# facebookresearch/flashy

Measured on AMD Instinct MI355X. Metric: img/sec, higher is better.
Workload: dtype bf16; 1 GPU; model=resnet18, dataset=cifar10-shaped, global_batch=64, img_size=32, num_classes=10, parallelism=dp1, mode=native-kernels, graph=True, channels_last=False

## Files before the change

flashy_amd/models/resnet_native.py:

```python
from __future__ import annotations

import typing as tp

import torch
from torch import nn

from .. import nn as fnn


class NativeBasicBlock(nn.Module):
    expansion = 1

    def __init__(self, cin: int, planes: int, stride: int = 1,
                 downsample: bool = False):
        super().__init__()
        self.conv1 = fnn.Conv2d(cin, planes, 3, stride, 1, feeds_bn=True)
        self.bn1 = fnn.BatchNorm2d(planes)
        self.conv2 = fnn.Conv2d(planes, planes, 3, 1, 1, feeds_bn=True)
        self.bn2 = fnn.BatchNorm2d(planes)
        if downsample:
            self.dconv = fnn.Conv2d(cin, planes, 1, stride, 0, feeds_bn=True)
            self.dbn = fnn.BatchNorm2d(planes)
        else:
            self.dconv = None
# ... 1 lines not shown
    def forward(self, x: torch.Tensor) -> torch.Tensor:
        if self.dconv is not None:
            identity = self.dbn(self.dconv(x))
        else:
            identity = x
        out = self.bn1(self.conv1(x), relu=True)
        out = self.conv2(out)
        return self.bn2(out, res=identity, relu=True)


class NativeBottleneck(nn.Module):
    expansion = 4

    def __init__(self, cin: int, planes: int, stride: int = 1,
                 downsample: bool = False):
        super().__init__()
        self.conv1 = fnn.Conv2d(cin, planes, 1, feeds_bn=True)
        self.bn1 = fnn.BatchNorm2d(planes)
        self.conv2 = fnn.Conv2d(planes, planes, 3, stride, 1, feeds_bn=True)
        self.bn2 = fnn.BatchNorm2d(planes)
        self.conv3 = fnn.Conv2d(planes, planes * 4, 1, feeds_bn=True)
        self.bn3 = fnn.BatchNorm2d(planes * 4)
        if downsample:
            self.dconv = fnn.Conv2d(cin, planes * 4, 1, stride, 0, feeds_bn=True)
            self.dbn = fnn.BatchNorm2d(planes * 4)
        else:
            self.dconv = None

    def forward(self, x: torch.Tensor) -> torch.Tensor:
        if self.dconv is not None:
            identity = self.dbn(self.dconv(x))
        else:
            identity = x
        out = self.bn1(self.conv1(x), relu=True)
        out = self.bn2(self.conv2(out), relu=True)
        out = self.conv3(out)
        return self.bn3(out, res=identity, relu=True)


class NativeResNet(nn.Module):

    def __init__(self, block: type, layers: tp.Sequence[int],
                 num_classes: int = 10, imagenet_stem: bool = False):
        super().__init__()
        self.imagenet_stem = imagenet_stem
        if imagenet_stem:
            self.stem_conv = fnn.Conv2d(3, 64, 7, 2, 3, input_grad=False)
            self.stem_pool = fnn.MaxPool2d(3, 2, 1)
        else:
            self.stem_conv = fnn.Conv2d(3, 64, 3, 1, 1, input_grad=False)
            self.stem_pool = None
        self.stem_bn = fnn.BatchNorm2d(64)
        self.inplanes = 64
        self.layer1 = self._make_layer(block, 64, layers[0])
        self.layer2 = self._make_layer(block, 128, layers[1], stride=2)
        self.layer3 = self._make_layer(block, 256, layers[2], stride=2)
        self.layer4 = self._make_layer(block, 512, layers[3], stride=2)
        self.fc = fnn.Linear(512 * block.expansion, num_classes)
        self._wt_cache = None

    def _make_layer(self, block: type, planes: int, n: int, stride: int = 1):
        downsample = stride != 1 or self.inplanes != planes * block.expansion
        blocks = [block(self.inplanes, planes, stride, downsample)]
        self.inplanes = planes * block.expansion
        blocks += [block(self.inplanes, planes) for _ in range(1, n)]
        return nn.Sequential(*blocks)

    def enable_wt_cache(self) -> "NativeResNet":
        cache = fnn.WtCache(self)
        self._wt_cache = cache if cache.active else None
        return self

    def forward(self, x: torch.Tensor) -> torch.Tensor:
        if self._wt_cache is not None and torch.is_grad_enabled():
            self._wt_cache.refresh()
        if x.shape[1] == 3:
            x = x.permute(0, 2, 3, 1).contiguous()
        if x.dtype != torch.bfloat16:
            x = x.to(torch.bfloat16)
        x = self.stem_bn(self.stem_conv(x), relu=True)
        if self.stem_pool is not None:
            x = self.stem_pool(x)
        x = self.layer4(self.layer3(self.layer2(self.layer1(x))))
        x = x.float().mean(dim=(1, 2))
        return self.fc(x)

    @torch.no_grad()
    def from_torch(self, twin: nn.Module) -> "NativeResNet":
        tsd = twin.state_dict()
        mapping = self._torch_key_map()
        for ours, theirs in mapping.items():
            dst = dict(self.state_dict())[ours]
            src = tsd[theirs]
            if src.dim() == 4:
                src = src.permute(0, 2, 3, 1).contiguous()
            dst.copy_(src)
        return self

    def _torch_key_map(self) -> tp.Dict[str, str]:
        m = {"stem_conv.weight": "stem.0.weight",
             "stem_bn.weight": "stem.1.weight",
             "stem_bn.bias": "stem.1.bias",
             "stem_bn.running_mean": "stem.1.running_mean",
             "stem_bn.running_var": "stem.1.running_var",
             "fc.weight": "fc.weight", "fc.bias": "fc.bias"}
        for name, mod in self.named_modules():
            if not isinstance(mod, (NativeBasicBlock, NativeBottleneck)):
                continue
            n_convs = 3 if isinstance(mod, NativeBottleneck) else 2
            for i in range(1, n_convs + 1):
                m[f"{name}.conv{i}.weight"] = f"{name}.conv{i}.weight"
                for suf in ("weight", "bias", "running_mean", "running_var"):
                    m[f"{name}.bn{i}.{suf}"] = f"{name}.bn{i}.{suf}"
            if mod.dconv is not None:
                m[f"{name}.dconv.weight"] = f"{name}.downsample.0.weight"
                for suf in ("weight", "bias", "running_mean", "running_var"):
                    m[f"{name}.dbn.{suf}"] = f"{name}.downsample.1.{suf}"
        return m


def native_resnet18(num_classes: int = 10,
                    imagenet_stem: bool = False) -> NativeResNet:
    return NativeResNet(NativeBasicBlock, [2, 2, 2, 2], num_classes,
                        imagenet_stem)


def native_resnet50(num_classes: int = 10,
                    imagenet_stem: bool = False) -> NativeResNet:
    return NativeResNet(NativeBottleneck, [3, 4, 6, 3], num_classes,
                        imagenet_stem)
```

flashy_amd/nn.py:

```python
from __future__ import annotations

import math
import os
import typing as tp

import torch
from torch import nn

from . import ops


def _weight_bf16(w: torch.Tensor) -> torch.Tensor:
    mirror = getattr(w, "_bf16_mirror", None)
    if mirror is not None:
        return mirror
    return w.detach().to(torch.bfloat16)


def _grad_target(p: torch.Tensor) -> tp.Tuple[torch.Tensor, bool]:
    if p.grad is not None and p.grad.is_contiguous():
        return p.grad, True
    return torch.zeros_like(p, memory_format=torch.contiguous_format), False


# ... 226 lines not shown
            torch.empty(in_channels, k, k, out_channels))
        fan_out = out_channels * k * k
        nn.init.normal_(self.weight, std=math.sqrt(2.0 / fan_out))

    def forward(self, x: torch.Tensor) -> torch.Tensor:
        return _ConvTransposeFn.apply(x, self.weight, self.stride,
                                      self.padding,
                                      self.input_grad and x.requires_grad)


_LINEAR_GEMM_CUTOFF = int(os.environ.get("FLASHY_LINEAR_CUTOFF", 1 << 23))


class _LinearFn(torch.autograd.Function):
    @staticmethod
    def forward(ctx, x: torch.Tensor, w: torch.Tensor,
                b: tp.Optional[torch.Tensor]):
        B, I = x.shape
        O = w.shape[0]
        big = 2 * B * I * O >= _LINEAR_GEMM_CUTOFF and x.dtype == torch.float32
        if big:
            x = x.contiguous()
            y = torch.addmm(b, x, w.t()) if b is not None else x.mm(w.t())
        else:
            y = x.new_empty((B, O))
            ops.linear_fwd(x.contiguous(), w, b, y)
        ctx.save_for_backward(x)
        ctx.refs = (w, b)
        ctx.big = big
        return y

    @staticmethod
    def backward(ctx, dy: torch.Tensor):
        (x,) = ctx.saved_tensors
        w, b = ctx.refs
        dy = dy.contiguous()
        dw = db = None
        need_w = ctx.needs_input_grad[1]
        need_b = b is not None and ctx.needs_input_grad[2]
        if ctx.big:
            if need_w:
                dw, w_direct = _grad_target(w)
                dw.addmm_(dy.t(), x)
                dw = None if w_direct else dw
            if need_b:
                db, b_direct = _grad_target(b)
                db.add_(dy.sum(0))
                db = None if b_direct else db
        elif need_w or need_b:
            dw, w_direct = _grad_target(w) if need_w \
                else (torch.empty_like(w), True)
            db, b_direct = (_grad_target(b) if need_b else (None, True))
            ops.linear_dw(x, dy, dw, db)
            dw = dw if need_w and not w_direct else None
            db = db if need_b and not b_direct else None
        dx = None
        if ctx.needs_input_grad[0]:
            if ctx.big:
                dx = dy.mm(w)
            else:
                dx = x.new_empty(x.shape)
                ops.linear_dx(dy, w, dx)
        return dx, dw, db


class Linear(nn.Module):

    def __init__(self, in_features: int, out_features: int, bias: bool = True):
        super().__init__()
        self.weight = nn.Parameter(torch.empty(out_features, in_features))
        bound = 1.0 / math.sqrt(in_features)
        nn.init.uniform_(self.weight, -bound, bound)
        self.bias: tp.Optional[nn.Parameter] = None
        if bias:
            self.bias = nn.Parameter(torch.empty(out_features))
            nn.init.uniform_(self.bias, -bound, bound)

    def forward(self, x: torch.Tensor) -> torch.Tensor:
        if x.device.type != "cuda":
            return torch.nn.functional.linear(x, self.weight, self.bias)
        return _LinearFn.apply(x, self.weight, self.bias)


class _MaxPoolFn(torch.autograd.Function):
    @staticmethod
    def forward(ctx, x: torch.Tensor, kernel: int, stride: int, pad: int):
        N, H, W, C = x.shape
        Ho = (H + 2 * pad - kernel) // stride + 1
        Wo = (W + 2 * pad - kernel) // stride + 1
        d = ops.ConvDims(N, H, W, C, C, kernel, kernel, Ho, Wo, stride, pad)
        y = x.new_empty((N, Ho, Wo, C))
        argmax = torch.empty(N * Ho * Wo * C, dtype=torch.uint8, device=x.device)
        ops.maxpool_fwd(x, y, argmax, d)
        ctx.save_for_backward(argmax)
        ctx.dims = d
        return y

    @staticmethod
    def backward(ctx, dy: torch.Tensor):
        (argmax,) = ctx.saved_tensors
        d: ops.ConvDims = ctx.dims
        dx = dy.new_empty((d.N, d.H, d.W, d.C))
        ops.maxpool_bwd(dy.contiguous(), argmax, dx, d)
        return dx, None, None, None


class MaxPool2d(nn.Module):

    def __init__(self, kernel_size: int, stride: int, padding: int = 0):
        super().__init__()
        self.kernel_size = kernel_size
        self.stride = stride
        self.padding = padding

    def forward(self, x: torch.Tensor) -> torch.Tensor:
        return _MaxPoolFn.apply(x, self.kernel_size, self.stride, self.padding)


class BatchNorm2d(nn.Module):

    def __init__(self, num_features: int, eps: float = 1e-5, momentum: float = 0.1):
        super().__init__()
        self.num_features = num_features
        self.eps = eps
        self.momentum = momentum
        self.weight = nn.Parameter(torch.ones(num_features))
        self.bias = nn.Parameter(torch.zeros(num_features))
        self.register_buffer("running_mean", torch.zeros(num_features))
        self.register_buffer("running_var", torch.ones(num_features))

    def forward(self, x: torch.Tensor,
                res: tp.Optional[torch.Tensor] = None,
                relu: bool = False, slope: float = 0.0) -> torch.Tensor:
        return _BnFn.apply(x, self.weight, self.bias, res, relu, slope, self)
```

flashy_amd/ops/__init__.py:

```python
from __future__ import annotations

import importlib.util
import os
import typing as tp
from pathlib import Path

import torch

_ext = None
_load_error: tp.Optional[str] = None


def _find_so() -> tp.Optional[Path]:
    for pattern in ("_hip_ops*.so",):
        hits = sorted(Path(__file__).parent.glob(pattern))
        if hits:
            return hits[0]
    return None


def load_extension():
    global _ext, _load_error
    if _ext is not None:
        return _ext
# ... 54 lines not shown
               p_bf16: tp.Optional[torch.Tensor] = None,
               step_dev: tp.Optional[torch.Tensor] = None) -> None:
    ext = require()
    assert p.is_contiguous() and g.is_contiguous()
    ext.fused_adam(p.data_ptr(), g.data_ptr(), m.data_ptr(), v.data_ptr(),
                   p_bf16.data_ptr() if p_bf16 is not None else 0,
                   step_dev.data_ptr() if step_dev is not None else 0,
                   p.numel(), lr, beta1, beta2, eps, wd, step, grad_scale,
                   adamw, _stream())


def adam_step_inc(step_dev: torch.Tensor) -> None:
    require().adam_step_inc(step_dev.data_ptr(), _stream())


def maxpool_fwd(x: torch.Tensor, y: torch.Tensor, argmax: torch.Tensor,
                d: "ConvDims") -> None:
    assert d.C % 8 == 0
    require().maxpool_fwd(x.data_ptr(), y.data_ptr(), argmax.data_ptr(), *d,
                          _stream())


def maxpool_bwd(dy: torch.Tensor, argmax: torch.Tensor, dx: torch.Tensor,
                d: "ConvDims") -> None:
    require().maxpool_bwd(dy.data_ptr(), argmax.data_ptr(), dx.data_ptr(), *d,
                          _stream())



class ConvDims(tp.NamedTuple):
    N: int; H: int; W: int; C: int
    K: int; R: int; S: int
    Ho: int; Wo: int
    stride: int; pad: int

    @staticmethod
    def infer(x: torch.Tensor, w: torch.Tensor, stride: int, pad: int) -> "ConvDims":
        N, H, W, C = x.shape
        K, R, S, Cw = w.shape
        assert C == Cw, (x.shape, w.shape)
        Ho = (H + 2 * pad - R) // stride + 1
        Wo = (W + 2 * pad - S) // stride + 1
        return ConvDims(N, H, W, C, K, R, S, Ho, Wo, stride, pad)


def _splitk_plan(M: int, ktiles: int, red_stages: int):
    if red_stages < 4:
        return 0
    blocks64 = ((M + 63) // 64) * ktiles
    if blocks64 >= 208:
        fill = 0
    else:
        fill = max(2, min((256 + blocks64 - 1) // max(1, blocks64),
                          red_stages // 2))
    longk = red_stages // 14 if red_stages >= 48 else 0
    zn = min(max(fill, longk), 8)
    return zn if zn >= 2 else 0


def conv_fwd(x: torch.Tensor, w: torch.Tensor, y: torch.Tensor, d: ConvDims,
             relu: bool = False,
             want_stats: bool = False) -> tp.Optional[tp.Tuple[torch.Tensor, int]]:
    ext = require()
    if d.C % 8 == 0:
        rsc = d.R * d.S * d.C
        assert d.K % 64 == 0 and rsc % 32 == 0, d
        M = d.N * d.Ho * d.Wo
        stages = (rsc + 63) // 64
        zn = 0 if ext.conv8_eligible(*d, False) else \
            _splitk_plan(M, d.K // 64, stages)
        if zn == 0 and stages >= 16 and not ext.conv8_eligible(*d, False):
            mt8 = (M + 255) // 256
            bn8 = 128 if d.K % 128 == 0 else 64
            tiles8 = mt8 * (d.K // bn8)
            if tiles8 and tiles8 < 160:
                zn = min(max(2, -(-160 // tiles8)), 8, stages // 8)
                zn = 0 if zn < 2 else zn
        if zn:
            spz = (stages + zn - 1) // zn
            zeff = (stages + spz - 1) // spz
            ws = torch.empty(zeff * M * d.K, dtype=torch.float32, device=x.device)
            ext.conv_fwd_splitk(x.data_ptr(), w.data_ptr(), ws.data_ptr(), *d,
                                spz, _stream())
            ext.splitk_combine(ws.data_ptr(), y.data_ptr(), M * d.K, zeff, relu,
                               _stream())
        else:
            stats = None
            bn_ptr = 0
            if want_stats:
                msplit = ext.conv_fwd_msplit(*d)
                partials = torch.empty(2 * d.K * msplit, dtype=torch.float32,
                                       device=x.device)
                stats = (partials, msplit)
                bn_ptr = partials.data_ptr()
            ext.conv_fwd(x.data_ptr(), w.data_ptr(), y.data_ptr(), *d, relu,
                         bn_ptr, _stream())
            return stats
    else:
        assert not relu
        M = d.N * d.Ho * d.Wo
        if d.C == 3 and d.K % 64 == 0 and d.R <= 8 and d.S <= 8 \
                and M >= 100_000:
            return _stem_fwd8(ext, x, w, y, d, want_stats)
        assert d.R * d.S * d.C <= 160 and d.K == 64, d
        ext.conv_stem_fwd(x.data_ptr(), w.data_ptr(), y.data_ptr(), *d, _stream())
    return None


def _stem_pad_x(ext, x: torch.Tensor, d: ConvDims) -> tp.Tuple[torch.Tensor, int, int]:
    Hp = (d.Ho - 1) * d.stride + 8
    Wp = (d.Wo - 1) * d.stride + 8
    xp = torch.empty(d.N, Hp, Wp, 4, dtype=torch.bfloat16, device=x.device)
    ext.stem_pad_x(x.data_ptr(), xp.data_ptr(), d.N, d.H, d.W, Hp, Wp, d.pad,
                   _stream())
    return xp, Hp, Wp


def _stem_fwd8(ext, x, w, y, d: ConvDims, want_stats: bool):
    xp, Hp, Wp = _stem_pad_x(ext, x, d)
    wp = torch.empty(d.K, 8, 8, 4, dtype=torch.bfloat16, device=x.device)
    ext.stem_pad_w(w.data_ptr(), wp.data_ptr(), d.K, d.R, d.S, _stream())
    M = d.N * d.Ho * d.Wo
    mtiles = (M + 255) // 256
    stats = None
    bn_ptr = 0
    if want_stats:
        partials = torch.empty(2 * d.K * mtiles, dtype=torch.float32,
                               device=x.device)
        stats = (partials, mtiles)
        bn_ptr = partials.data_ptr()
    ext.conv_fwd8_direct(xp.data_ptr(), wp.data_ptr(), y.data_ptr(),
                         d.N, Hp, Wp, 4, d.K, 8, 8, d.Ho, d.Wo, d.stride, 0,
                         False, bn_ptr, 64, mtiles, _stream())
    return stats


def conv_stem_dgrad(dout: torch.Tensor, w_krsc: torch.Tensor,
                    dx: torch.Tensor, d: ConvDims) -> None:
    assert d.C <= 8 and d.K == 64 and d.R * d.S * d.C <= 160, d
    require().conv_stem_dgrad(dout.data_ptr(), w_krsc.data_ptr(),
                              dx.data_ptr(), *d, _stream())


def conv_dgrad(dout: torch.Tensor, w_rsck: torch.Tensor, dx: torch.Tensor,
               d: ConvDims) -> None:
    ext = require()
    assert d.C % 64 == 0 and d.K % 32 == 0, d
    M = d.N * d.H * d.W
    rsk = d.R * d.S * d.K
    stages = (rsk + 63) // 64
    zn = 0 if ext.conv8_eligible(*d, True) else \
        _splitk_plan(M, d.C // 64, stages)
    if zn == 0 and stages >= 16 and d.stride == 1 \
            and not ext.conv8_eligible(*d, True):
        mt8 = (M + 255) // 256
        bn8 = 128 if d.C % 128 == 0 else 64
        tiles8 = mt8 * (d.C // bn8)
        if tiles8 and tiles8 < 160:
            zn = min(max(2, -(-160 // tiles8)), 8, stages // 8)
            zn = 0 if zn < 2 else zn
    if zn:
        spz = (stages + zn - 1) // zn
        zeff = (stages + spz - 1) // spz
        ws = torch.empty(zeff * M * d.C, dtype=torch.float32, device=dout.device)
        ext.conv_dgrad_splitk(dout.data_ptr(), w_rsck.data_ptr(), ws.data_ptr(),
                              *d, spz, _stream())
# ... 93 lines not shown
                  msplit: int, relu: bool, slope: float = 0.0) -> None:
    require().bn_bwd_reduce(dy.data_ptr(), y.data_ptr(), x.data_ptr(),
                            work.data_ptr(), dz_out.data_ptr(),
                            partials.data_ptr(), M, C, msplit, relu, slope,
                            _stream())


def bn_bwd_grads(partials, msplit: int, bsums, dgamma, dbeta, C: int) -> None:
    require().bn_bwd_grads(partials.data_ptr(), msplit, bsums.data_ptr(),
                           dgamma.data_ptr(), dbeta.data_ptr(), C, _stream())


def bn_bwd_apply(dz, x, work, bsums, dx, M: int, C: int) -> None:
    require().bn_bwd_apply(dz.data_ptr(), x.data_ptr(), work.data_ptr(),
                           bsums.data_ptr(), dx.data_ptr(), M, C, _stream())



def cross_entropy_fwd_bwd(logits: torch.Tensor, target: torch.Tensor,
                          dlogits: torch.Tensor, loss_sum: torch.Tensor,
                          loss_scale: float, grad_scale: float) -> None:
    ext = require()
    B, C = logits.shape
    assert logits.is_contiguous() and target.dtype == torch.int64
    ext.cross_entropy(logits.data_ptr(), target.data_ptr(), dlogits.data_ptr(),
                      loss_sum.data_ptr(), B, C, loss_scale, grad_scale,
                      _is_bf16(logits), _stream())


def bce_logits_fwd_bwd(x: torch.Tensor, dx: torch.Tensor,
                       loss_sum: torch.Tensor, target: float,
                       loss_scale: float, grad_scale: float) -> None:
    ext = require()
    assert x.is_contiguous()
    ext.bce_logits(x.data_ptr(), dx.data_ptr(), loss_sum.data_ptr(), x.numel(),
                   target, loss_scale, grad_scale, _is_bf16(x), _stream())


def mse_fwd_bwd(x: torch.Tensor, t: torch.Tensor, dx: torch.Tensor,
                loss_sum: torch.Tensor, loss_scale: float,
                grad_scale: float) -> None:
    ext = require()
    assert x.is_contiguous() and t.is_contiguous() and x.dtype == t.dtype
    ext.mse(x.data_ptr(), t.data_ptr(), dx.data_ptr(), loss_sum.data_ptr(),
            x.numel(), loss_scale, grad_scale, _is_bf16(x), _stream())


def accuracy_count(logits: torch.Tensor, target: torch.Tensor,
                   out: torch.Tensor) -> None:
    ext = require()
    B, C = logits.shape
    assert logits.is_contiguous() and target.dtype == torch.int64
    ext.accuracy(logits.data_ptr(), target.data_ptr(), out.data_ptr(), B, C,
                 _is_bf16(logits), _stream())



def linear_fwd(x: torch.Tensor, w: torch.Tensor,
               b: tp.Optional[torch.Tensor], y: torch.Tensor) -> None:
    ext = require()
    B, I = x.shape
    O = w.shape[0]
    assert x.dtype == torch.float32 and w.shape == (O, I)
    ext.linear_fwd(x.data_ptr(), w.data_ptr(),
                   b.data_ptr() if b is not None else 0,
                   y.data_ptr(), B, I, O, _stream())


def linear_dx(dy: torch.Tensor, w: torch.Tensor, dx: torch.Tensor) -> None:
    ext = require()
    B, O = dy.shape
    I = w.shape[1]
    ext.linear_dx(dy.data_ptr(), w.data_ptr(), dx.data_ptr(), B, I, O,
                  _stream())


def linear_dw(x: torch.Tensor, dy: torch.Tensor, dw: torch.Tensor,
              db: tp.Optional[torch.Tensor]) -> None:
    ext = require()
    B, I = x.shape
    O = dy.shape[1]
    ext.linear_dw(x.data_ptr(), dy.data_ptr(), dw.data_ptr(),
                  db.data_ptr() if db is not None else 0, B, I, O, _stream())
```

flashy_amd/ops/csrc/conv_fwd.hip:

```cpp

#include "conv_common.h"

template <int BM, bool RELU, bool SPLITK, int SUBS = 2, int BN = CONV_BN>
__global__ void __launch_bounds__(CONV_THREADS)
k_conv_fwd(const uint16_t* __restrict__ x, const uint16_t* __restrict__ w,
           uint16_t* __restrict__ y, float* __restrict__ ws_out,
           float* __restrict__ bn_ws, ConvDims d, int stages_per_split) {
    constexpr int WAVES_M = BM >= 64 ? 2 : 1;
    constexpr int WAVES_N = 4 / WAVES_M;
    constexpr int MF = BM / WAVES_M / 16;
    constexpr int NF = BN / WAVES_N / 16;
    constexpr int BK2 = SUBS * CONV_BK;
    constexpr int CHUNKS = BM * (BK2 / 8);
    constexpr int CPT = (CHUNKS + CONV_THREADS - 1) / CONV_THREADS;

    const int rsc = d.R * d.S * d.C;
    const int64_t M = (int64_t)d.N * d.Ho * d.Wo;
    const int tid = threadIdx.x;
    const int lane = tid & 63;
    const int wid = tid >> 6;
    const int wave_m = WAVES_M == 1 ? 0 : (wid >> 1);
    const int wave_n = WAVES_M == 1 ? wid : (wid & 1);
    unsigned bx = blockIdx.x;
    if ((gridDim.x & 7) == 0) bx = (bx & 7) * (gridDim.x >> 3) + (bx >> 3);
// ... 126 lines not shown
#pragma unroll
        for (int nf = 0; nf < NF; ++nf)
#pragma unroll
            for (int rr = 0; rr < 4; ++rr) {
                const int64_t row = out_row0 + mf * 16 + rr;
                if (row < M) {
                    float v = acc[mf][nf][rr];
                    if (SPLITK) {
                        ws_out[((int64_t)blockIdx.z * M + row) * d.K +
                               out_col0 + nf * 16] = v;
                    } else {
                        if (RELU) v = fmaxf(v, 0.f);
                        y[row * d.K + out_col0 + nf * 16] = f32_to_bf16(v);
                    }
                }
            }

    if (!SPLITK && bn_ws != nullptr) {
        float* sred = reinterpret_cast<float*>(A_lds);
#pragma unroll
        for (int nf = 0; nf < NF; ++nf) {
            float s = 0.f, s2 = 0.f;
#pragma unroll
            for (int mf = 0; mf < MF; ++mf)
#pragma unroll
                for (int rr = 0; rr < 4; ++rr) {
                    float v = acc[mf][nf][rr];
                    if (RELU) v = fmaxf(v, 0.f);
                    s += v;
                    s2 = fmaf(v, v, s2);
                }
            s += __shfl_xor(s, 16, 64);
            s += __shfl_xor(s, 32, 64);
            s2 += __shfl_xor(s2, 16, 64);
            s2 += __shfl_xor(s2, 32, 64);
            if (lane < 16) {
                const int colL = wave_n * (BN / WAVES_N) + nf * 16 + lane;
                sred[wave_m * BN + colL] = s;
                sred[(WAVES_M + wave_m) * BN + colL] = s2;
            }
        }
        __syncthreads();
        if (tid < BN) {
            float s = 0.f, s2 = 0.f;
#pragma unroll
            for (int wm = 0; wm < WAVES_M; ++wm) {
                s += sred[wm * BN + tid];
                s2 += sred[(WAVES_M + wm) * BN + tid];
            }
            const int c = col0 + tid;
            bn_ws[((int64_t)c) * gridDim.x + blockIdx.x] = s;
            bn_ws[((int64_t)d.K + c) * gridDim.x + blockIdx.x] = s2;
        }
    }
}

__global__ void __launch_bounds__(256)
k_splitk_combine(const float* __restrict__ ws, uint16_t* __restrict__ out,
                 int64_t total, int zn, int relu) {
    const int64_t stride = (int64_t)gridDim.x * blockDim.x;
    for (int64_t i = (int64_t)blockIdx.x * blockDim.x + threadIdx.x;
         i * 4 < total; i += stride) {
        float4 acc = *reinterpret_cast<const float4*>(ws + i * 4);
        for (int z = 1; z < zn; ++z) {
            const float4 v = *reinterpret_cast<const float4*>(
                ws + (int64_t)z * total + i * 4);
            acc.x += v.x; acc.y += v.y; acc.z += v.z; acc.w += v.w;
        }
        if (relu) {
            acc.x = fmaxf(acc.x, 0.f); acc.y = fmaxf(acc.y, 0.f);
            acc.z = fmaxf(acc.z, 0.f); acc.w = fmaxf(acc.w, 0.f);
        }
        ushort4 o;
        o.x = f32_to_bf16(acc.x); o.y = f32_to_bf16(acc.y);
        o.z = f32_to_bf16(acc.z); o.w = f32_to_bf16(acc.w);
        *reinterpret_cast<ushort4*>(out + i * 4) = o;
    }
}

extern "C" void launch_splitk_combine(const void* ws, void* out, int64_t total,
                                      int zn, int relu, hipStream_t stream) {
    k_splitk_combine<<<ew_grid(total / 4, 256, 2), 256, 0, stream>>>(
        (const float*)ws, (uint16_t*)out, total, zn, relu);
}

static void pick_tile(int64_t M, int K, int* bm_out, int* bn_out) {
    if (K % 128 == 0 && (M + 127) / 128 * (K / 128) >= 208) {
        *bm_out = 128;
        *bn_out = 128;
        return;
    }
    *bn_out = 64;
    for (int bm : {128, 64}) {
        if ((M + bm - 1) / bm * (K / 64) >= 208) { *bm_out = bm; return; }
    }
    *bm_out = 32;
}

#include <cstdlib>
static int conv_subs() {
    static int v = [] {
        const char* e = getenv("FLASHY_CONV_SUBS");
        return (e && e[0] == '1') ? 1 : 2;
    }();
    return v;
}

extern "C" int conv_fwd8_plan(ConvDims d, int* bn_out);
extern "C" void launch_conv_fwd8(const void* x, const void* w, void* y,
                                 ConvDims d, int relu, void* bn_ws, int bn,
                                 int mtiles, hipStream_t stream);
extern "C" int conv1x1_mloop_plan(ConvDims d, int* bn_out, int* gridx_out);
extern "C" int conv_dedup_plan(ConvDims d, int* bn_out, int* tpi_out,
                               int* rows_out, int* elems_out);
extern "C" void launch_conv_dedup(const void* x, const void* w, void* y,
                                  ConvDims d, int relu, void* bn_ws, int bn,
                                  int tpi, int rows, int lds_elems,
                                  hipStream_t stream);
extern "C" void launch_conv1x1_mloop(const void* x, const void* w, void* y,
                                     ConvDims d, int relu, void* bn_ws,
                                     int bn, int gridx, int mtiles,
                                     hipStream_t stream);

extern "C" int conv_fwd_msplit(ConvDims d) {
    int bn8, gx;
    {
        int tpi, rows, elems;
        const int gd = conv_dedup_plan(d, &bn8, &tpi, &rows, &elems);
        if (gd) return gd;
    }
    const int mtl = conv1x1_mloop_plan(d, &bn8, &gx);
    if (mtl) return 2 * mtl;
    const int mt8 = conv_fwd8_plan(d, &bn8);
    if (mt8) return mt8;
    const int64_t M = (int64_t)d.N * d.Ho * d.Wo;
    int bm, bn;
    pick_tile(M, d.K, &bm, &bn);
    return (int)((M + bm - 1) / bm);
}

extern "C" void launch_conv_fwd(const void* x, const void* w, void* y,
                                ConvDims d, int relu, void* bn_ws,
                                hipStream_t stream) {
    int bn8, gx;
    {
        int tpi, rows, elems;
        const int gd = conv_dedup_plan(d, &bn8, &tpi, &rows, &elems);
        if (gd) {
            launch_conv_dedup(x, w, y, d, relu, bn_ws, bn8, tpi, rows,
                              elems, stream);
            return;
        }
    }
    const int mtl = conv1x1_mloop_plan(d, &bn8, &gx);
    if (mtl) {
        launch_conv1x1_mloop(x, w, y, d, relu, bn_ws, bn8, gx, mtl, stream);
        return;
    }
    const int mt8 = conv_fwd8_plan(d, &bn8);
    if (mt8) {
        launch_conv_fwd8(x, w, y, d, relu, bn_ws, bn8, mt8, stream);
        return;
    }
    const int64_t M = (int64_t)d.N * d.Ho * d.Wo;
    int bm, bn;
    pick_tile(M, d.K, &bm, &bn);
// ... 516 lines not shown
```

flashy_amd/ops/csrc/ext.cpp:

```cpp

#include <hip/hip_runtime.h>
#include <pybind11/pybind11.h>

#include <cstdint>
#include <stdexcept>

namespace py = pybind11;

struct ConvDims {
    int N, H, W, C;
    int K, R, S;
    int Ho, Wo;
    int stride, pad;
};

extern "C" {
void launch_conv_fwd(const void* x, const void* w, void* y, ConvDims d,
                     int relu, void* bn_ws, hipStream_t stream);
int conv_fwd_msplit(ConvDims d);
int conv_fwd8_plan(ConvDims d, int* bn_out);
int conv_dgrad8_plan(ConvDims d, int* bn_out);
void launch_conv_fwd8(const void* x, const void* w, void* y, ConvDims d,
                      int relu, void* bn_ws, int bn, int mtiles,
                      hipStream_t stream);
void launch_stem_pad_x(const void* x, void* xp, int64_t N, int H, int W,
                       int Hp, int Wp, int pad, hipStream_t stream);
void launch_stem_pad_w(const void* w, void* wp, int K, int R, int S,
                       hipStream_t stream);
void launch_stem_unpad_dw(const void* dwp, void* dw, int K, int R, int S,
                          hipStream_t stream);
void launch_conv_stem_fwd(const void* x, const void* w, void* y, ConvDims d,
                          hipStream_t stream);
void launch_conv_stem_wgrad(const void* x, const void* dout, void* dw,
                            ConvDims d, hipStream_t stream);
void launch_conv_stem_dgrad(const void* dout, const void* w, void* dx,
                            ConvDims d, hipStream_t stream);
void launch_conv_dgrad(const void* dout, const void* w_rsck, void* dx,
                       ConvDims d, hipStream_t stream);
void launch_conv_fwd_splitk(const void* x, const void* w, void* ws, ConvDims d,
                            int zn, hipStream_t stream);
void launch_conv_dgrad_splitk(const void* dout, const void* w_rsck, void* ws,
                              ConvDims d, int zn, hipStream_t stream);
void launch_splitk_combine(const void* ws, void* out, int64_t total, int zn,
                           int relu, hipStream_t stream);
void launch_weight_transpose(const void* w, void* wt, int K, int rsc,
                             hipStream_t stream);
void launch_weight_transpose_batched(const void* src, void* dst,
                                     const void* meta, int n_convs,
                                     int64_t max_elems, hipStream_t stream);
void launch_conv_wgrad(const void* x, const void* dout, void* dw, ConvDims d,
                       int n_splits, hipStream_t stream);
void launch_bn_stats(const void* x, void* partials, int64_t M, int C,
                     int msplit, hipStream_t stream);
void launch_bn_finalize(const void* partials, int msplit, const void* gamma,
                        const void* beta, void* running_mean,
                        void* running_var, void* work, int64_t M, int C,
                        float eps, float momentum, int update_running,
                        hipStream_t stream);
void launch_bn_apply(const void* x, const void* res, void* y, const void* work,
                     int64_t M, int C, int relu, float slope,
                     hipStream_t stream);
void launch_bn_bwd_reduce(const void* dy, const void* y, const void* x,
                          const void* work, void* dz_out, void* partials,
                          int64_t M, int C, int msplit, int relu, float slope,
                          hipStream_t stream);
void launch_bn_bwd_grads(const void* partials, int msplit, void* bsums,
                         void* dgamma, void* dbeta, int C, hipStream_t stream);
void launch_bn_bwd_apply(const void* dz, const void* x, const void* work,
                         const void* bsums, void* dx, int64_t M, int C,
                         hipStream_t stream);
void launch_fused_sgd(void* p, const void* g, void* m, void* p_bf16, int64_t n,
                      float lr, float momentum, float wd, float grad_scale,
                      int nesterov, hipStream_t stream);
void launch_fused_adam(void* p, const void* g, void* m, void* v, void* p_bf16,
                       void* step_dev, int64_t n, float lr, float beta1,
                       float beta2, float eps, float wd, int64_t step,
                       float grad_scale, int adamw, hipStream_t stream);
void launch_adam_step_inc(void* p, hipStream_t stream);
void launch_maxpool_fwd(const void* x, void* y, void* argmax, ConvDims d,
                        hipStream_t stream);
void launch_maxpool_bwd(const void* dy, const void* argmax, void* dx,
                        ConvDims d, hipStream_t stream);
void launch_cross_entropy(const void* logits, const void* target, void* dlogits,
                          void* loss_sum, int64_t B, int64_t C,
                          float loss_scale, float grad_scale, int is_bf16,
                          hipStream_t stream);
void launch_mse(const void* x, const void* t, void* dx, void* loss_sum,
                int64_t n, float loss_scale, float grad_scale, int is_bf16,
                hipStream_t stream);
void launch_accuracy(const void* logits, const void* target, void* out,
                     int64_t B, int64_t C, int is_bf16, hipStream_t stream);
void launch_linear_fwd(const void* x, const void* w, const void* b, void* y,
                       int64_t B, int64_t I, int64_t O, hipStream_t stream);
void launch_linear_dx(const void* dy, const void* w, void* dx, int64_t B,
                      int64_t I, int64_t O, hipStream_t stream);
void launch_linear_dw(const void* x, const void* dy, void* dw, void* db,
                      int64_t B, int64_t I, int64_t O, hipStream_t stream);
void launch_bce_logits(const void* x, void* dx, void* loss_sum, int64_t n,
                       float target, float loss_scale, float grad_scale,
                       int is_bf16, hipStream_t stream);
}

static void check_last() {
    hipError_t err = hipGetLastError();
    if (err != hipSuccess)
        throw std::runtime_error(std::string("HIP launch failed: ") +
                                 hipGetErrorString(err));
}

static hipStream_t as_stream(uintptr_t s) { return reinterpret_cast<hipStream_t>(s); }

static ConvDims make_dims(int N, int H, int W, int C, int K, int R, int S,
                          int Ho, int Wo, int stride, int pad) {
    return ConvDims{N, H, W, C, K, R, S, Ho, Wo, stride, pad};
}

PYBIND11_MODULE(_hip_ops, m) {
    m.doc() = "flashy_amd gfx950 kernels";
    m.attr("ARCH") = "gfx950";

    m.def("conv_fwd",
          [](uintptr_t x, uintptr_t w, uintptr_t y, int N, int H, int W, int C,
             int K, int R, int S, int Ho, int Wo, int stride, int pad,
             bool relu, uintptr_t bn_ws, uintptr_t stream) {
              launch_conv_fwd((const void*)x, (const void*)w, (void*)y,
                              make_dims(N, H, W, C, K, R, S, Ho, Wo, stride, pad),
                              relu ? 1 : 0, (void*)bn_ws, as_stream(stream));
// ... 36 lines not shown
              check_last();
          });

    m.def("conv8_eligible",
          [](int N, int H, int W, int C, int K, int R, int S, int Ho, int Wo,
             int stride, int pad, bool dgrad) {
              int bn = 0;
              ConvDims d = make_dims(N, H, W, C, K, R, S, Ho, Wo, stride, pad);
              return (dgrad ? conv_dgrad8_plan(d, &bn)
                            : conv_fwd8_plan(d, &bn)) > 0;
          });

    m.def("conv_fwd_msplit",
          [](int N, int H, int W, int C, int K, int R, int S, int Ho, int Wo,
             int stride, int pad) {
              return conv_fwd_msplit(
                  make_dims(N, H, W, C, K, R, S, Ho, Wo, stride, pad));
          });
    m.def("conv_stem_fwd",
          [](uintptr_t x, uintptr_t w, uintptr_t y, int N, int H, int W, int C,
             int K, int R, int S, int Ho, int Wo, int stride, int pad,
             uintptr_t stream) {
              launch_conv_stem_fwd((const void*)x, (const void*)w, (void*)y,
                                   make_dims(N, H, W, C, K, R, S, Ho, Wo, stride, pad),
                                   as_stream(stream));
              check_last();
          });
    m.def("conv_stem_wgrad",
          [](uintptr_t x, uintptr_t dout, uintptr_t dw, int N, int H, int W,
             int C, int K, int R, int S, int Ho, int Wo, int stride, int pad,
             uintptr_t stream) {
              launch_conv_stem_wgrad((const void*)x, (const void*)dout,
                                     (void*)dw,
                                     make_dims(N, H, W, C, K, R, S, Ho, Wo, stride, pad),
                                     as_stream(stream));
              check_last();
          });
    m.def("conv_stem_dgrad",
          [](uintptr_t dout, uintptr_t w, uintptr_t dx, int N, int H, int W,
             int C, int K, int R, int S, int Ho, int Wo, int stride, int pad,
             uintptr_t stream) {
              launch_conv_stem_dgrad((const void*)dout, (const void*)w,
                                     (void*)dx,
                                     make_dims(N, H, W, C, K, R, S, Ho, Wo, stride, pad),
                                     as_stream(stream));
              check_last();
          });
    m.def("conv_dgrad",
          [](uintptr_t dout, uintptr_t w_rsck, uintptr_t dx, int N, int H,
             int W, int C, int K, int R, int S, int Ho, int Wo, int stride,
             int pad, uintptr_t stream) {
              launch_conv_dgrad((const void*)dout, (const void*)w_rsck,
                                (void*)dx,
                                make_dims(N, H, W, C, K, R, S, Ho, Wo, stride, pad),
                                as_stream(stream));
              check_last();
          });
    m.def("conv_fwd_splitk",
          [](uintptr_t x, uintptr_t w, uintptr_t ws, int N, int H, int W,
             int C, int K, int R, int S, int Ho, int Wo, int stride, int pad,
             int zn, uintptr_t stream) {
              launch_conv_fwd_splitk((const void*)x, (const void*)w, (void*)ws,
                                     make_dims(N, H, W, C, K, R, S, Ho, Wo, stride, pad),
                                     zn, as_stream(stream));
              check_last();
          });
    m.def("conv_dgrad_splitk",
          [](uintptr_t dout, uintptr_t w_rsck, uintptr_t ws, int N, int H,
             int W, int C, int K, int R, int S, int Ho, int Wo, int stride,
             int pad, int zn, uintptr_t stream) {
              launch_conv_dgrad_splitk((const void*)dout, (const void*)w_rsck,
                                       (void*)ws,
                                       make_dims(N, H, W, C, K, R, S, Ho, Wo, stride, pad),
                                       zn, as_stream(stream));
              check_last();
          });
    m.def("splitk_combine",
          [](uintptr_t ws, uintptr_t out, int64_t total, int zn, bool relu,
             uintptr_t stream) {
              launch_splitk_combine((const void*)ws, (void*)out, total, zn,
                                    relu ? 1 : 0, as_stream(stream));
              check_last();
          });
    m.def("weight_transpose",
          [](uintptr_t w, uintptr_t wt, int K, int rsc, uintptr_t stream) {
              launch_weight_transpose((const void*)w, (void*)wt, K, rsc,
                                      as_stream(stream));
              check_last();
          });
    m.def("weight_transpose_batched",
          [](uintptr_t src, uintptr_t dst, uintptr_t meta, int n_convs,
             int64_t max_elems, uintptr_t stream) {
              launch_weight_transpose_batched((const void*)src, (void*)dst,
                                              (const void*)meta, n_convs,
                                              max_elems, as_stream(stream));
              check_last();
          });
    m.def("conv_wgrad",
          [](uintptr_t x, uintptr_t dout, uintptr_t dw, int N, int H, int W,
             int C, int K, int R, int S, int Ho, int Wo, int stride, int pad,
             int n_splits, uintptr_t stream) {
              launch_conv_wgrad((const void*)x, (const void*)dout, (void*)dw,
                                make_dims(N, H, W, C, K, R, S, Ho, Wo, stride, pad),
                                n_splits, as_stream(stream));
              check_last();
          });
    m.def("bn_stats",
          [](uintptr_t x, uintptr_t partials, int64_t M, int C, int msplit,
             uintptr_t stream) {
              launch_bn_stats((const void*)x, (void*)partials, M, C, msplit,
                              as_stream(stream));
              check_last();
          });
    m.def("bn_finalize",
          [](uintptr_t partials, int msplit, uintptr_t gamma, uintptr_t beta,
             uintptr_t rmean, uintptr_t rvar, uintptr_t work, int64_t M, int C,
             float eps, float momentum, bool update_running, uintptr_t stream) {
              launch_bn_finalize((const void*)partials, msplit,
                                 (const void*)gamma, (const void*)beta,
                                 (void*)rmean, (void*)rvar, (void*)work, M, C,
                                 eps, momentum, update_running ? 1 : 0,
                                 as_stream(stream));
              check_last();
          });
    m.def("bn_apply",
          [](uintptr_t x, uintptr_t res, uintptr_t y, uintptr_t work, int64_t M,
             int C, bool relu, float slope, uintptr_t stream) {
              launch_bn_apply((const void*)x, (const void*)res, (void*)y,
                              (const void*)work, M, C, relu ? 1 : 0, slope,
                              as_stream(stream));
              check_last();
          });
    m.def("bn_bwd_reduce",
          [](uintptr_t dy, uintptr_t y, uintptr_t x, uintptr_t work,
             uintptr_t dz_out, uintptr_t partials, int64_t M, int C,
             int msplit, bool relu, float slope, uintptr_t stream) {
              launch_bn_bwd_reduce((const void*)dy, (const void*)y,
                                   (const void*)x, (const void*)work,
                                   (void*)dz_out, (void*)partials, M, C,
                                   msplit, relu ? 1 : 0, slope,
                                   as_stream(stream));
              check_last();
          });
    m.def("bn_bwd_grads",
          [](uintptr_t partials, int msplit, uintptr_t bsums, uintptr_t dgamma,
             uintptr_t dbeta, int C, uintptr_t stream) {
              launch_bn_bwd_grads((const void*)partials, msplit, (void*)bsums,
                                  (void*)dgamma, (void*)dbeta, C,
                                  as_stream(stream));
              check_last();
          });
    m.def("bn_bwd_apply",
          [](uintptr_t dz, uintptr_t x, uintptr_t work, uintptr_t bsums,
             uintptr_t dx, int64_t M, int C, uintptr_t stream) {
              launch_bn_bwd_apply((const void*)dz, (const void*)x,
                                  (const void*)work, (const void*)bsums,
                                  (void*)dx, M, C, as_stream(stream));
              check_last();
          });

    m.def("fused_sgd",
          [](uintptr_t p, uintptr_t g, uintptr_t mom, uintptr_t p_bf16,
             int64_t n, float lr, float momentum, float wd, float grad_scale,
             bool nesterov, uintptr_t stream) {
              launch_fused_sgd((void*)p, (const void*)g, (void*)mom,
                               (void*)p_bf16, n, lr, momentum, wd, grad_scale,
// ... 20 lines not shown
          [](uintptr_t x, uintptr_t y, uintptr_t argmax, int N, int H, int W,
             int C, int K, int R, int S, int Ho, int Wo, int stride, int pad,
             uintptr_t stream) {
              launch_maxpool_fwd((const void*)x, (void*)y, (void*)argmax,
                                 make_dims(N, H, W, C, K, R, S, Ho, Wo, stride, pad),
                                 as_stream(stream));
              check_last();
          });
    m.def("maxpool_bwd",
          [](uintptr_t dy, uintptr_t argmax, uintptr_t dx, int N, int H, int W,
             int C, int K, int R, int S, int Ho, int Wo, int stride, int pad,
             uintptr_t stream) {
              launch_maxpool_bwd((const void*)dy, (const void*)argmax,
                                 (void*)dx,
                                 make_dims(N, H, W, C, K, R, S, Ho, Wo, stride, pad),
                                 as_stream(stream));
              check_last();
          });

    m.def("cross_entropy",
          [](uintptr_t logits, uintptr_t target, uintptr_t dlogits,
             uintptr_t loss_sum, int64_t B, int64_t C, float loss_scale,
             float grad_scale, bool is_bf16, uintptr_t stream) {
              launch_cross_entropy((const void*)logits, (const void*)target,
                                   (void*)dlogits, (void*)loss_sum, B, C,
                                   loss_scale, grad_scale, is_bf16 ? 1 : 0,
                                   as_stream(stream));
              check_last();
          });

    m.def("bce_logits",
          [](uintptr_t x, uintptr_t dx, uintptr_t loss_sum, int64_t n,
             float target, float loss_scale, float grad_scale, bool is_bf16,
             uintptr_t stream) {
              launch_bce_logits((const void*)x, (void*)dx, (void*)loss_sum, n,
                                target, loss_scale, grad_scale,
                                is_bf16 ? 1 : 0, as_stream(stream));
              check_last();
          });

    m.def("mse",
          [](uintptr_t x, uintptr_t t, uintptr_t dx, uintptr_t loss_sum,
             int64_t n, float loss_scale, float grad_scale, bool is_bf16,
             uintptr_t stream) {
              launch_mse((const void*)x, (const void*)t, (void*)dx,
                         (void*)loss_sum, n, loss_scale, grad_scale,
                         is_bf16 ? 1 : 0, as_stream(stream));
              check_last();
          });

    m.def("accuracy",
          [](uintptr_t logits, uintptr_t target, uintptr_t out, int64_t B,
             int64_t C, bool is_bf16, uintptr_t stream) {
              launch_accuracy((const void*)logits, (const void*)target,
                              (void*)out, B, C, is_bf16 ? 1 : 0,
                              as_stream(stream));
              check_last();
          });

    m.def("linear_fwd",
          [](uintptr_t x, uintptr_t w, uintptr_t b, uintptr_t y, int64_t B,
             int64_t I, int64_t O, uintptr_t stream) {
              launch_linear_fwd((const void*)x, (const void*)w,
                                (const void*)b, (void*)y, B, I, O,
                                as_stream(stream));
              check_last();
          });

    m.def("linear_dx",
          [](uintptr_t dy, uintptr_t w, uintptr_t dx, int64_t B, int64_t I,
             int64_t O, uintptr_t stream) {
              launch_linear_dx((const void*)dy, (const void*)w, (void*)dx, B,
                               I, O, as_stream(stream));
              check_last();
          });

    m.def("linear_dw",
          [](uintptr_t x, uintptr_t dy, uintptr_t dw, uintptr_t db, int64_t B,
             int64_t I, int64_t O, uintptr_t stream) {
              launch_linear_dw((const void*)x, (const void*)dy, (void*)dw,
                               (void*)db, B, I, O, as_stream(stream));
              check_last();
          });
}
```

Measured before the change: 28950 img/s.

## Fuse global average pool with FC head and split-K combine with BN stats

Replaces the float cast, mean and separate linear layer at the end of the ResNet with one fused pool+FC forward kernel, plus dedicated backward kernels for dW/db and a broadcast dX. It also adds a split-K combine kernel that writes the bf16 conv output and BatchNorm partial statistics in one pass, avoiding a separate stats read. The aim is fewer launches and less memory traffic on the small head and on split-K convs that feed BatchNorm. The cost is more custom kernels with LDS-size asserts, and the split-K path now returns partials early, which relies on callers handling that shape.

```diff
diff --git a/flashy_amd/models/resnet_native.py b/flashy_amd/models/resnet_native.py
--- a/flashy_amd/models/resnet_native.py
+++ b/flashy_amd/models/resnet_native.py
@@ -107,8 +107,7 @@
         if self.stem_pool is not None:
             x = self.stem_pool(x)
         x = self.layer4(self.layer3(self.layer2(self.layer1(x))))
-        x = x.float().mean(dim=(1, 2))
-        return self.fc(x)
+        return fnn.pool_linear(x, self.fc.weight, self.fc.bias)
 
     @torch.no_grad()
     def from_torch(self, twin: nn.Module) -> "NativeResNet":
diff --git a/flashy_amd/nn.py b/flashy_amd/nn.py
--- a/flashy_amd/nn.py
+++ b/flashy_amd/nn.py
@@ -332,6 +332,82 @@
         return _LinearFn.apply(x, self.weight, self.bias)
 
 
+class _PoolLinearFn(torch.autograd.Function):
+
+    @staticmethod
+    def forward(ctx, x: torch.Tensor, w: torch.Tensor,
+                b: tp.Optional[torch.Tensor]):
+        x = x.contiguous()
+        N, H, W, C = x.shape
+        pooled = torch.empty((N, C), dtype=torch.float32, device=x.device)
+        y = torch.empty((N, w.shape[0]), dtype=torch.float32, device=x.device)
+        ops.pool_linear_fwd(x, w, b, pooled, y)
+        ctx.save_for_backward(pooled)
+        ctx.refs = (w, b)
+        ctx.x_shape = x.shape
+        return y
+
+    @staticmethod
+    def backward(ctx, dy: torch.Tensor):
+        (pooled,) = ctx.saved_tensors
+        w, b = ctx.refs
+        dy = dy.contiguous()
+        dw = db = None
+        need_w = ctx.needs_input_grad[1]
+        need_b = b is not None and ctx.needs_input_grad[2]
+        if need_w or need_b:
+            dw, w_direct = _grad_target(w) if need_w else (None, True)
+            db, b_direct = _grad_target(b) if need_b else (None, True)
+            ops.head_dw(pooled, dy, dw, db)
+            dw = None if w_direct else dw
+            db = None if b_direct else db
+        dx = None
+        if ctx.needs_input_grad[0]:
+            dx = torch.empty(ctx.x_shape, dtype=torch.bfloat16,
+                             device=dy.device)
+            ops.head_dx(dy, w, dx)
+        return dx, dw, db
+
+
+class _PoolFn(torch.autograd.Function):
+
+    @staticmethod
+    def forward(ctx, x: torch.Tensor):
+        x = x.contiguous()
+        N, H, W, C = x.shape
+        pooled = torch.empty((N, C), dtype=torch.float32, device=x.device)
+        ops.pool_linear_fwd(x, None, None, pooled, None)
+        ctx.x_shape = x.shape
+        return pooled
+
+    @staticmethod
+    def backward(ctx, g: torch.Tensor):
+        dx = torch.empty(ctx.x_shape, dtype=torch.bfloat16, device=g.device)
+        ops.head_dx(g.contiguous(), None, dx)
+        return dx
+
+
+def pool_linear(x: torch.Tensor, weight: torch.Tensor,
+                bias: tp.Optional[torch.Tensor]) -> torch.Tensor:
+    if x.device.type != "cuda":
+        return torch.nn.functional.linear(x.float().mean(dim=(1, 2)),
+                                          weight, bias)
+    N, C = x.shape[0], x.shape[3]
+    if 2 * N * C * weight.shape[0] < _LINEAR_GEMM_CUTOFF:
+        return _PoolLinearFn.apply(x, weight, bias)
+    return _LinearFn.apply(_PoolFn.apply(x), weight, bias)
+
+
+class PoolLinearHead(nn.Module):
+
+    def __init__(self, in_features: int, out_features: int, bias: bool = True):
+        super().__init__()
+        self.fc = Linear(in_features, out_features, bias)
+
+    def forward(self, x: torch.Tensor) -> torch.Tensor:
+        return pool_linear(x, self.fc.weight, self.fc.bias)
+
+
 class _MaxPoolFn(torch.autograd.Function):
     @staticmethod
     def forward(ctx, x: torch.Tensor, kernel: int, stride: int, pad: int):
diff --git a/flashy_amd/ops/__init__.py b/flashy_amd/ops/__init__.py
--- a/flashy_amd/ops/__init__.py
+++ b/flashy_amd/ops/__init__.py
@@ -160,6 +160,15 @@
             ws = torch.empty(zeff * M * d.K, dtype=torch.float32, device=x.device)
             ext.conv_fwd_splitk(x.data_ptr(), w.data_ptr(), ws.data_ptr(), *d,
                                 spz, _stream())
+            if want_stats:
+                assert not relu, "a conv feeding BatchNorm has no fused ReLU"
+                msplit = bn_msplit(M, d.K)
+                partials = torch.empty(2 * d.K * msplit, dtype=torch.float32,
+                                       device=x.device)
+                ext.splitk_combine_stats(ws.data_ptr(), y.data_ptr(),
+                                         partials.data_ptr(), M, d.K, zeff,
+                                         msplit, _stream())
+                return partials, msplit
             ext.splitk_combine(ws.data_ptr(), y.data_ptr(), M * d.K, zeff, relu,
                                _stream())
         else:
@@ -419,3 +428,50 @@
     O = dy.shape[1]
     ext.linear_dw(x.data_ptr(), dy.data_ptr(), dw.data_ptr(),
                   db.data_ptr() if db is not None else 0, B, I, O, _stream())
+
+
+
+def pool_linear_fwd(x: torch.Tensor, w: tp.Optional[torch.Tensor],
+                    b: tp.Optional[torch.Tensor], pooled: torch.Tensor,
+                    y: tp.Optional[torch.Tensor]) -> None:
+    ext = require()
+    N, H, W, C = x.shape
+    assert x.dtype == torch.bfloat16 and x.is_contiguous() and C % 8 == 0
+    assert pooled.dtype == torch.float32 and pooled.shape == (N, C)
+    assert C * max(1, 2048 // C) * 4 <= 65536, f"C={C} exceeds the LDS row"
+    O = 0
+    if w is not None:
+        O = w.shape[0]
+        assert w.dtype == torch.float32 and w.shape == (O, C) \
+            and w.is_contiguous() and y is not None and y.shape == (N, O)
+    ext.pool_fc_fwd(x.data_ptr(), w.data_ptr() if w is not None else 0,
+                    b.data_ptr() if b is not None else 0, pooled.data_ptr(),
+                    y.data_ptr() if y is not None else 0, N, H * W, C, O,
+                    _stream())
+
+
+def head_dw(pooled: torch.Tensor, dy: torch.Tensor,
+            dw: tp.Optional[torch.Tensor],
+            db: tp.Optional[torch.Tensor]) -> None:
+    B, C = pooled.shape
+    O = dy.shape[1]
+    assert dy.dtype == torch.float32 and dy.is_contiguous()
+    require().head_dw(pooled.data_ptr(), dy.data_ptr(),
+                      dw.data_ptr() if dw is not None else 0,
+                      db.data_ptr() if db is not None else 0, B, C, O,
+                      _stream())
+
+
+def head_dx(dy: torch.Tensor, w: tp.Optional[torch.Tensor],
+            dx: torch.Tensor) -> None:
+    N, H, W, C = dx.shape
+    assert dx.dtype == torch.bfloat16 and dx.is_contiguous() and C % 8 == 0
+    assert dy.dtype == torch.float32 and dy.is_contiguous()
+    O = 0
+    if w is not None:
+        O = w.shape[0]
+        assert w.shape == (O, C) and w.is_contiguous() and dy.shape == (N, O)
+    else:
+        assert dy.shape == (N, C)
+    require().head_dx(dy.data_ptr(), w.data_ptr() if w is not None else 0,
+                      dx.data_ptr(), N, H * W, C, O, _stream())
diff --git a/flashy_amd/ops/csrc/conv_fwd.hip b/flashy_amd/ops/csrc/conv_fwd.hip
--- a/flashy_amd/ops/csrc/conv_fwd.hip
+++ b/flashy_amd/ops/csrc/conv_fwd.hip
@@ -232,6 +232,69 @@
                                       int zn, int relu, hipStream_t stream) {
     k_splitk_combine<<<ew_grid(total / 4, 256, 2), 256, 0, stream>>>(
         (const float*)ws, (uint16_t*)out, total, zn, relu);
+}
+
+__global__ void __launch_bounds__(256)
+k_splitk_combine_stats(const float* __restrict__ ws, uint16_t* __restrict__ out,
+                       float* __restrict__ partials, int64_t M, int K, int zn,
+                       int msplit, int m_per_block) {
+    const int c8 = (threadIdx.x & 7) * 8;
+    const int mlane = threadIdx.x >> 3;
+    const int cbase = blockIdx.x * 64;
+    const int64_t m0 = (int64_t)blockIdx.y * m_per_block;
+    const int64_t m1 = min(m0 + (int64_t)m_per_block, M);
+    const int64_t slice = M * K;
+    float s[8] = {}, s2[8] = {};
+    for (int64_t m = m0 + mlane; m < m1; m += 32) {
+        const int64_t off = m * K + cbase + c8;
+        float4 a = *reinterpret_cast<const float4*>(ws + off);
+        float4 b = *reinterpret_cast<const float4*>(ws + off + 4);
+        for (int z = 1; z < zn; ++z) {
+            const float4 va = *reinterpret_cast<const float4*>(
+                ws + (int64_t)z * slice + off);
+            const float4 vb = *reinterpret_cast<const float4*>(
+                ws + (int64_t)z * slice + off + 4);
+            a.x += va.x; a.y += va.y; a.z += va.z; a.w += va.w;
+            b.x += vb.x; b.y += vb.y; b.z += vb.z; b.w += vb.w;
+        }
+        const float v[8] = {a.x, a.y, a.z, a.w, b.x, b.y, b.z, b.w};
+        short8 o;
+#pragma unroll
+        for (int j = 0; j < 8; ++j) {
+            const uint16_t r = f32_to_bf16(v[j]);
+            const float vr = bf16_to_f32(r);
+            s[j] += vr;
+            s2[j] = fmaf(vr, vr, s2[j]);
+            ((uint16_t*)&o)[j] = r;
+        }
+        *reinterpret_cast<short8*>(out + off) = o;
+    }
+    __shared__ float red[2][32][64];
+#pragma unroll
+    for (int j = 0; j < 8; ++j) {
+        red[0][mlane][c8 + j] = s[j];
+        red[1][mlane][c8 + j] = s2[j];
+    }
+    __syncthreads();
+    const int c = threadIdx.x & 63;
+    const int which = threadIdx.x >> 6;
+    if (which < 2) {
+        float acc = 0.f;
+#pragma unroll 8
+        for (int i = 0; i < 32; ++i) acc += red[which][i][c];
+        partials[((int64_t)which * K + cbase + c) * msplit + blockIdx.y] = acc;
+    }
+}
+
+extern "C" void launch_splitk_combine_stats(const void* ws, void* out,
+                                            void* partials, int64_t M, int K,
+                                            int zn, int msplit,
+                                            hipStream_t stream) {
+    const int mpb = (int)((M + msplit - 1) / msplit);
+    dim3 grid((unsigned)(K / 64), (unsigned)msplit);
+    k_splitk_combine_stats<<<grid, 256, 0, stream>>>(
+        (const float*)ws, (uint16_t*)out, (float*)partials, M, K, zn, msplit,
+        mpb);
 }
 
 static void pick_tile(int64_t M, int K, int* bm_out, int* bn_out) {
diff --git a/flashy_amd/ops/csrc/ext.cpp b/flashy_amd/ops/csrc/ext.cpp
--- a/flashy_amd/ops/csrc/ext.cpp
+++ b/flashy_amd/ops/csrc/ext.cpp
@@ -43,6 +43,16 @@
                               ConvDims d, int zn, hipStream_t stream);
 void launch_splitk_combine(const void* ws, void* out, int64_t total, int zn,
                            int relu, hipStream_t stream);
+void launch_splitk_combine_stats(const void* ws, void* out, void* partials,
+                                 int64_t M, int K, int zn, int msplit,
+                                 hipStream_t stream);
+void launch_pool_fc_fwd(const void* x, const void* w, const void* b,
+                        void* pooled, void* y, int N, int HW, int C, int O,
+                        hipStream_t stream);
+void launch_head_dw(const void* pooled, const void* dy, void* dw, void* db,
+                    int B, int C, int O, hipStream_t stream);
+void launch_head_dx(const void* dy, const void* w, void* dx, int N, int HW,
+                    int C, int O, hipStream_t stream);
 void launch_weight_transpose(const void* w, void* wt, int K, int rsc,
                              hipStream_t stream);
 void launch_weight_transpose_batched(const void* src, void* dst,
@@ -245,6 +255,14 @@
                                     relu ? 1 : 0, as_stream(stream));
               check_last();
           });
+    m.def("splitk_combine_stats",
+          [](uintptr_t ws, uintptr_t out, uintptr_t partials, int64_t M, int K,
+             int zn, int msplit, uintptr_t stream) {
+              launch_splitk_combine_stats((const void*)ws, (void*)out,
+                                          (void*)partials, M, K, zn, msplit,
+                                          as_stream(stream));
+              check_last();
+          });
     m.def("weight_transpose",
           [](uintptr_t w, uintptr_t wt, int K, int rsc, uintptr_t stream) {
               launch_weight_transpose((const void*)w, (void*)wt, K, rsc,
@@ -431,4 +449,29 @@
                                (void*)db, B, I, O, as_stream(stream));
               check_last();
           });
+
+    m.def("pool_fc_fwd",
+          [](uintptr_t x, uintptr_t w, uintptr_t b, uintptr_t pooled,
+             uintptr_t y, int N, int HW, int C, int O, uintptr_t stream) {
+              launch_pool_fc_fwd((const void*)x, (const void*)w,
+                                 (const void*)b, (void*)pooled, (void*)y, N,
+                                 HW, C, O, as_stream(stream));
+              check_last();
+          });
+
+    m.def("head_dw",
+          [](uintptr_t pooled, uintptr_t dy, uintptr_t dw, uintptr_t db,
+             int B, int C, int O, uintptr_t stream) {
+              launch_head_dw((const void*)pooled, (const void*)dy, (void*)dw,
+                             (void*)db, B, C, O, as_stream(stream));
+              check_last();
+          });
+
+    m.def("head_dx",
+          [](uintptr_t dy, uintptr_t w, uintptr_t dx, int N, int HW, int C,
+             int O, uintptr_t stream) {
+              launch_head_dx((const void*)dy, (const void*)w, (void*)dx, N,
+                             HW, C, O, as_stream(stream));
+              check_last();
+          });
 }
diff --git a/flashy_amd/ops/csrc/head.hip b/flashy_amd/ops/csrc/head.hip
--- /dev/null
+++ b/flashy_amd/ops/csrc/head.hip
@@ -0,0 +1,160 @@
+
+#include "common.h"
+
+__global__ void __launch_bounds__(256)
+k_pool_fc_fwd(const uint16_t* __restrict__ x, const float* __restrict__ w,
+              const float* __restrict__ bias, float* __restrict__ pooled,
+              float* __restrict__ y, int HW, int C, int O, int cols, int rl) {
+    extern __shared__ float part[];
+    const int n = blockIdx.x;
+    const int col = threadIdx.x % cols;
+    const int row = threadIdx.x / cols;
+    const uint16_t* xn = x + (int64_t)n * HW * C;
+    if (row < rl) {
+        for (int c8 = col * 8; c8 < C; c8 += cols * 8) {
+            float s[8] = {};
+#pragma unroll 4
+            for (int hw = row; hw < HW; hw += rl) {
+                const short8 v8 = *reinterpret_cast<const short8*>(
+                    xn + (int64_t)hw * C + c8);
+#pragma unroll
+                for (int j = 0; j < 8; ++j)
+                    s[j] += bf16_to_f32(((const uint16_t*)&v8)[j]);
+            }
+#pragma unroll
+            for (int j = 0; j < 8; ++j) part[row * C + c8 + j] = s[j];
+        }
+    }
+    __syncthreads();
+    const float inv = 1.f / (float)HW;
+    for (int c = threadIdx.x; c < C; c += 256) {
+        float acc = part[c];
+        for (int r = 1; r < rl; ++r) acc += part[r * C + c];
+        acc *= inv;
+        part[c] = acc;
+        pooled[(int64_t)n * C + c] = acc;
+    }
+    if (w == nullptr) return;
+    __syncthreads();
+    const int lane = threadIdx.x & 63;
+    for (int o = threadIdx.x >> 6; o < O; o += 4) {
+        const float* wr = w + (int64_t)o * C;
+        float acc = 0.f;
+        for (int c = lane * 4; c < C; c += 256) {
+            const float4 wv = *reinterpret_cast<const float4*>(wr + c);
+            acc = fmaf(part[c], wv.x, acc);
+            acc = fmaf(part[c + 1], wv.y, acc);
+            acc = fmaf(part[c + 2], wv.z, acc);
+            acc = fmaf(part[c + 3], wv.w, acc);
+        }
+        acc = wave_sum(acc);
+        if (lane == 0)
+            y[(int64_t)n * O + o] = acc + (bias != nullptr ? bias[o] : 0.f);
+    }
+}
+
+__global__ void __launch_bounds__(256)
+k_head_dw(const float* __restrict__ pooled, const float* __restrict__ dy,
+          float* __restrict__ dw, float* __restrict__ db,
+          int B, int C, int O) {
+    const int idx = blockIdx.x * 256 + threadIdx.x;
+    if (idx >= O * C) return;
+    const int o = idx / C, c = idx - o * C;
+    if (dw != nullptr) {
+        float acc = 0.f;
+#pragma unroll 8
+        for (int n = 0; n < B; ++n)
+            acc = fmaf(dy[(int64_t)n * O + o], pooled[(int64_t)n * C + c], acc);
+        dw[idx] += acc;
+    }
+    if (db != nullptr && c == 0) {
+        float bs = 0.f;
+        for (int n = 0; n < B; ++n) bs += dy[(int64_t)n * O + o];
+        db[o] += bs;
+    }
+}
+
+__global__ void __launch_bounds__(256)
+k_head_dx(const float* __restrict__ dy, const float* __restrict__ w,
+          uint16_t* __restrict__ dx, int HW, int C, int O, int cols, int rl,
+          int hw_per_block) {
+    const int n = blockIdx.x;
+    const int col = threadIdx.x % cols;
+    const int row = threadIdx.x / cols;
+    if (row >= rl) return;
+    const int hw0 = blockIdx.y * hw_per_block;
+    const int hw1 = min(hw0 + hw_per_block, HW);
+    const float inv = 1.f / (float)HW;
+    uint16_t* dxn = dx + (int64_t)n * HW * C;
+    for (int c8 = col * 8; c8 < C; c8 += cols * 8) {
+        float g[8];
+        if (w != nullptr) {
+#pragma unroll
+            for (int j = 0; j < 8; ++j) g[j] = 0.f;
+            for (int o = 0; o < O; ++o) {
+                const float d = dy[(int64_t)n * O + o];
+                const float4 w0 = *reinterpret_cast<const float4*>(
+                    w + (int64_t)o * C + c8);
+                const float4 w1 = *reinterpret_cast<const float4*>(
+                    w + (int64_t)o * C + c8 + 4);
+                g[0] = fmaf(d, w0.x, g[0]); g[1] = fmaf(d, w0.y, g[1]);
+                g[2] = fmaf(d, w0.z, g[2]); g[3] = fmaf(d, w0.w, g[3]);
+                g[4] = fmaf(d, w1.x, g[4]); g[5] = fmaf(d, w1.y, g[5]);
+                g[6] = fmaf(d, w1.z, g[6]); g[7] = fmaf(d, w1.w, g[7]);
+            }
+        } else {
+            const float4 g0 = *reinterpret_cast<const float4*>(
+                dy + (int64_t)n * C + c8);
+            const float4 g1 = *reinterpret_cast<const float4*>(
+                dy + (int64_t)n * C + c8 + 4);
+            g[0] = g0.x; g[1] = g0.y; g[2] = g0.z; g[3] = g0.w;
+            g[4] = g1.x; g[5] = g1.y; g[6] = g1.z; g[7] = g1.w;
+        }
+        short8 out;
+#pragma unroll
+        for (int j = 0; j < 8; ++j)
+            ((uint16_t*)&out)[j] = f32_to_bf16(g[j] * inv);
+        for (int hw = hw0 + row; hw < hw1; hw += rl)
+            *reinterpret_cast<short8*>(dxn + (int64_t)hw * C + c8) = out;
+    }
+}
+
+static inline void head_geometry(int C, int* cols, int* rl) {
+    const int noct = C / 8;
+    *cols = noct < 256 ? noct : 256;
+    *rl = 256 / *cols;
+}
+
+extern "C" void launch_pool_fc_fwd(const void* x, const void* w, const void* b,
+                                   void* pooled, void* y, int N, int HW, int C,
+                                   int O, hipStream_t stream) {
+    int cols, rl;
+    head_geometry(C, &cols, &rl);
+    const size_t lds = (size_t)rl * C * sizeof(float);
+    k_pool_fc_fwd<<<(unsigned)N, 256, lds, stream>>>(
+        (const uint16_t*)x, (const float*)w, (const float*)b, (float*)pooled,
+        (float*)y, HW, C, O, cols, rl);
+}
+
+extern "C" void launch_head_dw(const void* pooled, const void* dy, void* dw,
+                               void* db, int B, int C, int O,
+                               hipStream_t stream) {
+    k_head_dw<<<(unsigned)((O * C + 255) / 256), 256, 0, stream>>>(
+        (const float*)pooled, (const float*)dy, (float*)dw, (float*)db, B, C,
+        O);
+}
+
+extern "C" void launch_head_dx(const void* dy, const void* w, void* dx, int N,
+                               int HW, int C, int O, hipStream_t stream) {
+    int cols, rl;
+    head_geometry(C, &cols, &rl);
+    int split = (256 + N - 1) / N;
+    const int max_split = (HW + rl - 1) / rl;
+    if (split > max_split) split = max_split;
+    if (split < 1) split = 1;
+    const int hpb = (HW + split - 1) / split;
+    dim3 grid((unsigned)N, (unsigned)((HW + hpb - 1) / hpb));
+    k_head_dx<<<grid, 256, 0, stream>>>(
+        (const float*)dy, (const float*)w, (uint16_t*)dx, HW, C, O, cols, rl,
+        hpb);
+}
```

Measured after the change: 30060 img/s, median of 6. +3.8%, better.
